# Digital-Defiance/node-fhe-accelerate

Hardware: AMD Instinct MI355X
Metric: NTTs/s at degree 16384 (batched, forward NTT + pointwise modmul) (higher is better)
Workload: dtype u64 (32-bit Shoup/Montgomery lanes for q<2^30); 1 GPU; C3: N=16384 forward NTT + modmul, batch 65536 per GPU, q=132120577; n=16384, batch_per_gpu=65536, global_batch=65536, q=132120577, parallelism=batch-sharded x1, no data-path collective

## Files before the change

node-fhe-accelerate_amd/csrc/fhe_arith.hpp:

```cpp
#pragma once
#ifndef FHE_NS
#define FHE_NS fhe
#endif
#include <hip/hip_runtime.h>
#include <stdint.h>

namespace FHE_NS {

__device__ __forceinline__ uint32_t mulhi(uint32_t a, uint32_t b) { return __umulhi(a, b); }
#ifndef FHE_MULHI64
#define FHE_MULHI64 3
#endif
__device__ __forceinline__ uint64_t mulhi(uint64_t a, uint64_t b) {
#if FHE_MULHI64 == 4
    const uint32_t a0 = (uint32_t)a, a1 = (uint32_t)(a >> 32), b0 = (uint32_t)b, b1 = (uint32_t)(b >> 32);
    const uint64_t m1 = (uint64_t)a1 * b0 + (uint64_t)__umulhi(a0, b0);
    const uint64_t m2 = (uint64_t)a0 * b1 + (uint64_t)(uint32_t)m1;
    const uint64_t h = (uint64_t)a1 * b1 + (m1 >> 32);
    return h + (m2 >> 32);
#elif FHE_MULHI64 == 3
    const uint32_t a0 = (uint32_t)a, a1 = (uint32_t)(a >> 32), b0 = (uint32_t)b, b1 = (uint32_t)(b >> 32);
    const uint64_t m1 = (uint64_t)a1 * b0 + __umulhi(a0, b0);
    uint64_t m2, cy;
    asm("v_mad_u64_u32 %0, %1, %2, %3, %4" : "=&v"(m2), "=&s"(cy) : "v"(a0), "v"(b1), "v"(m1));
// ... 158 lines not shown
        u32x2 cc;
        cc.x = c;
        uint64_t r, cy;
        asm("v_mad_u64_u32 %0, %1, %2, %3, %4" : "=&v"(r), "=&s"(cy) : "v"(a), "v"(b), "v"(cc));
        (void)cy;
        return (uint32_t)r;
    }
    static __device__ __forceinline__ uint32_t madlo_s(uint32_t a, uint32_t b, uint32_t c) {
        typedef uint32_t u32x2 __attribute__((ext_vector_type(2)));
        u32x2 cc;
        cc.x = c;
        uint64_t r, cy;
        asm("v_mad_u64_u32 %0, %1, %2, %3, %4" : "=&v"(r), "=&s"(cy) : "v"(a), "s"(b), "v"(cc));
        (void)cy;
        return (uint32_t)r;
    }
    template <int SP = 0>
    __device__ __forceinline__ W shoup(W x, Tw<W> t) const { return shoup<true, SP>(x, t.w, t.wp); }
    template <int SP = 0>
    __device__ __forceinline__ W shoup_inv(W x, Tw<W> t) const { return shoup<false, SP>(x, t.w, t.wp); }

    __device__ __forceinline__ W mont(W a, W b) const {
        W lo = a * b;
        W hi = mulhi(a, b);
        if constexpr (sizeof(W) == 8 && FHE_U64_NOVCC) {
            const W m = lo * (W(0) - qinv);
            return (W)sub_add64(hi, mulhi(m, q), (uint64_t)q + 1);
        } else {
            W m = lo * qinv;
            return hi + mulhi(m, q) + (lo != 0 ? W(1) : W(0));
        }
    }

    __device__ __forceinline__ W red2q(W x) const { return redk(x, q2); }
    __device__ __forceinline__ W red1q(W x) const { return redk(x, q); }
    static __device__ __forceinline__ W redk(W x, W k) {
        if constexpr (sizeof(W) == 8 && FHE_U64_NOVCC) {
            return (W)redk64(x, k);
        } else if constexpr (sizeof(W) == 8 && FHE_RED64_BORROW) {
            W d;
            return __builtin_sub_overflow(x, k, &d) ? x : d;
        } else {
            return umin(x, W(x - k));
        }
    }
    __device__ __forceinline__ W canon4(W x) const { return red1q(red2q(x)); }

    __device__ __forceinline__ W shoup_neg(W y, Tw<W> t) const {
        const W h = mulhi(y, t.wp);
        typedef uint32_t u32x2 __attribute__((ext_vector_type(2)));
        u32x2 c;
        c.x = y * t.w;
        uint64_t r, cy;
        asm("v_mad_u64_u32 %0, %1, %2, %3, %4" : "=&v"(r), "=&s"(cy) : "v"(h), "s"(q), "v"(c));
        (void)cy;
        return (W)r;
    }
    template <int SP = 0>
    __device__ __forceinline__ void ct(W &x, W &y, Tw<W> t) const {
        W a = red2q(x);
        if constexpr (sizeof(W) == 4 && FHE_NEG_FWD_TW) {
            const W nb = shoup_neg(y, t);
            x = a - nb;
            y = a + nb + q2;
        } else {
            W b = shoup<SP>(y, t);
// ... 19 lines not shown
        }
    }
    template <int SP = 0>
    __device__ __forceinline__ void ct_rscale(W &x, W &y, Scale<W> r) const {
        W a = shoup<SP>(x, r.a);
        W b = shoup<SP>(y, r.b);
        x = a + b;
        y = sub2q(a, b);
    }
    __device__ __forceinline__ void ct_unit(W &x, W &y) const {
        const W a = red2q(x), b = red2q(y);
        x = a + b;
        y = sub2q(a, b);
    }
    __device__ __forceinline__ void gs_unit(W &x, W &y) const {
        const W s = x + y, d = sub2q(x, y);
        x = red2q(s);
        y = red2q(d);
    }
    template <int SP = 0>
    __device__ __forceinline__ void gs(W &x, W &y, Tw<W> t) const {
        W s = x + y;
        W d = sub2q(x, y);
        x = red2q(s);
        y = shoup_inv<SP>(d, t);
    }
    template <int SP = 0>
    __device__ __forceinline__ void gs_scaled(W &x, W &y, Scale<W> ninv) const {
        W s = x + y;
        W d = sub2q(x, y);
        x = shoup_inv<SP>(s, ninv.a);
        y = shoup_inv<SP>(d, ninv.b);
    }
};

__device__ __forceinline__ uint64_t mod64_slow(uint64_t x, uint64_t q, uint64_t mu) {
    if (q >> 63) return x >= q ? x - q : x;
    uint64_t r = x - __umul64hi(x, mu) * q;
    return r >= q ? r - q : r;
}

__device__ __forceinline__ uint64_t wmont(uint64_t a, uint64_t b, uint64_t q, uint64_t qinv) {
    const uint64_t lo = a * b, hi = __umul64hi(a, b);
    const uint64_t mh = __umul64hi(lo * qinv, q);
    const uint64_t s = hi + mh;
    const bool c1 = s < hi;
    const uint64_t s2 = s + (lo != 0);
    const bool c2 = s2 < s;
    return (c1 || c2 || s2 >= q) ? s2 - q : s2;
}
__device__ __forceinline__ uint64_t wadd(uint64_t a, uint64_t b, uint64_t q) {
    const uint64_t s = a + b;
    return (s < a || s >= q) ? s - q : s;
}
__device__ __forceinline__ uint64_t wsub(uint64_t a, uint64_t b, uint64_t q) { return a >= b ? a - b : a - b + q; }
template <typename W>
__device__ __forceinline__ W load_lazy(uint64_t x, uint64_t lim, uint64_t q, uint64_t mu) {
    if (x >= lim) x = mod64_slow(x, q, mu);
    return W(x);
}

}
```

node-fhe-accelerate_amd/csrc/fhe_gpu.cpp:

```cpp
#include <hip/hip_runtime.h>

#include <algorithm>
#include <cstdlib>
#include <cstdio>
#include <cstring>
#include <mutex>
#include <thread>
#include <string>
#include <vector>

#include "../../include/fhe_gpu.h"
#include "fhe_internal.hpp"
#include "keygen.hpp"
#include "build_id.h"

using u64 = uint64_t;
using u32 = uint32_t;
using u128 = unsigned __int128;

namespace {

thread_local std::string g_err;

int fail(int code, const std::string &msg) {
// ... 772 lines not shown
            if (e != hipSuccess) { rc = hip_fail(e, "hipMalloc(big-N scratch)"); break; }
        }
    }
    if (rc == FHE_OK) {
        hipError_t e = hipStreamCreateWithFlags(&c->own_stream, hipStreamNonBlocking);
        if (e != hipSuccess) rc = hip_fail(e, "hipStreamCreate");
    }
    if (rc == FHE_OK) {
        const char *kv = std::getenv("FHE_POOL_KEEP_MB");
        const uint64_t keep_mb = kv ? std::strtoull(kv, nullptr, 10) : 8192;
        hipMemPool_t pool = nullptr;
        if (keep_mb && hipDeviceGetDefaultMemPool(&pool, device) == hipSuccess && pool) {
            uint64_t keep = keep_mb << 20;
            (void)hipMemPoolSetAttribute(pool, hipMemPoolAttrReleaseThreshold, &keep);
        }
        (void)hipGetLastError();
    }
    if (rc != FHE_OK) {
        free_tables(c);
        delete c;
        return rc;
    }
    c->stream = c->own_stream;
    c->plan.logn = logn;
    c->plan.word = c->word;
    {
        int cus = 0;
        if (hipDeviceGetAttribute(&cus, hipDeviceAttributeMultiprocessorCount, device) != hipSuccess || cus <= 0) cus = 256;
        (void)hipGetLastError();
        c->plan.cus = cus;
    }
    c->plan.wide = c->wide;
    c->plan.lazy = c->word == 32 && (u128)(4 + 2 * logn) * q <= ((u128)1 << 32);
    {
        const char *u = std::getenv("FHE_UNIT_TW");
        c->plan.compat = c->mode == FHE_MODE_COMPAT && !(u && u[0] == '0');
    }
    c->plan.stream = c->stream;
    c->plan.big_sync = &c->big_sync;
    *out = c;
    return FHE_OK;
}

int fhe_ctx_create_multi(uint32_t n, uint64_t q, int mode, const int *devices, int ndev, fhe_ctx **out) {
    if (!out) return fail(FHE_ERR_INVALID_ARG, "null out");
    *out = nullptr;
    if (!devices || ndev < 1) return fail(FHE_ERR_INVALID_ARG, "at least one device required");
    fhe_ctx *m = new fhe_ctx();
    for (int i = 0; i < ndev; ++i) {
        fhe_ctx *s = nullptr;
        const int rc = fhe_ctx_create(n, q, mode, devices[i], &s);
        if (rc != FHE_OK) {
            const std::string msg = g_err;
            fhe_ctx_destroy(m);
            return fail(rc, msg);
        }
        m->subs.push_back(s);
    }
    const fhe_ctx *s0 = m->subs[0];
    m->n = s0->n; m->logn = s0->logn; m->q = s0->q; m->psi = s0->psi; m->psi_inv = s0->psi_inv;
    m->inv_n = s0->inv_n; m->mode = s0->mode; m->device = s0->device; m->word = s0->word;
    m->fwd_tw = s0->fwd_tw; m->inv_tw = s0->inv_tw;
    m->stream = s0->stream;
    *out = m;
    return FHE_OK;
}
// ... 647 lines not shown
    FHE_TRY(hs.map(where, lwe_b, batch * 8, 1));
    FHE_TRY(hs.map(where, values, batch * 8, 2));
    FHE_TRY(hs.map(where, phase, batch * 8, 2));
    HIP_TRY(FHE_NS::launch_lwe_decrypt(q, t, sk, dim, lwe_a, lwe_b, values, phase, batch, s), "lwe decrypt kernel");
    return where == FHE_HOST ? hs.finish() : FHE_OK;
}

struct fhe_rns_ctx {
    std::vector<fhe_ctx *> limbs;
    void *tab = nullptr;
    FHE_NS::ModConsts *mtab = nullptr;
};

int fhe_rns_ctx_create(uint32_t n, const uint64_t *moduli, uint32_t count, int mode, int device, fhe_rns_ctx **out) {
    if (!out) return fail(FHE_ERR_INVALID_ARG, "null out");
    *out = nullptr;
    if (count == 0 || !moduli) return fail(FHE_ERR_INVALID_ARG, "At least one modulus required");
    fhe_rns_ctx *r = new fhe_rns_ctx();
    for (uint32_t i = 0; i < count; ++i) {
        fhe_ctx *c = nullptr;
        const int rc = fhe_ctx_create(n, moduli[i], mode, device, &c);
        if (rc != FHE_OK) {
            const std::string msg = g_err;
            fhe_rns_ctx_destroy(r);
            return fail(rc, msg);
        }
        if (!r->limbs.empty()) fhe_ctx_set_stream(c, r->limbs[0]->stream);
        r->limbs.push_back(c);
    }
    const fhe_ctx *c0 = r->limbs[0];
    bool one = !c0->plan.wide && (int)c0->logn <= FHE_NS::kMaxFusedLogN;
    for (const fhe_ctx *c : r->limbs)
        one = one && !c->plan.wide && c->plan.word == c0->plan.word && c->plan.lazy == c0->plan.lazy &&
              c->logn == c0->logn && c->device == c0->device;
    if (one) {
        DeviceGuard g(c0->device);
        const size_t L = r->limbs.size();
        std::vector<FHE_NS::ModConsts> mc(L);
        for (size_t i = 0; i < L; ++i) mc[i] = mod_consts(r->limbs[i]->q);
        std::vector<char> at;
        if (c0->plan.word == 32) {
            at.resize(L * sizeof(FHE_NS::NttArgs<uint32_t>));
            for (size_t i = 0; i < L; ++i)
                std::memcpy(at.data() + i * sizeof(FHE_NS::NttArgs<uint32_t>), &r->limbs[i]->plan.a32,
                            sizeof(FHE_NS::NttArgs<uint32_t>));
        } else {
            at.resize(L * sizeof(FHE_NS::NttArgs<uint64_t>));
            for (size_t i = 0; i < L; ++i)
                std::memcpy(at.data() + i * sizeof(FHE_NS::NttArgs<uint64_t>), &r->limbs[i]->plan.a64,
                            sizeof(FHE_NS::NttArgs<uint64_t>));
        }
        hipError_t e = hipMalloc(&r->tab, at.size());
        if (e == hipSuccess) e = hipMalloc((void **)&r->mtab, L * sizeof(FHE_NS::ModConsts));
        if (e == hipSuccess) e = hipMemcpy(r->tab, at.data(), at.size(), hipMemcpyHostToDevice);
        if (e == hipSuccess) e = hipMemcpy(r->mtab, mc.data(), L * sizeof(FHE_NS::ModConsts), hipMemcpyHostToDevice);
        if (e != hipSuccess) {
            fhe_rns_ctx_destroy(r);
            return hip_fail(e, "hipMalloc(RNS limb tables)");
        }
    }
    *out = r;
    return FHE_OK;
}

void fhe_rns_ctx_destroy(fhe_rns_ctx *r) {
    if (!r) return;
    if (r->tab || r->mtab) {
// ... 713 lines not shown
```

node-fhe-accelerate_amd/csrc/fhe_internal.hpp:

```cpp
#pragma once
#include <hip/hip_runtime.h>
#include <stddef.h>
#include <stdint.h>

#include <mutex>

#include "ntt_core.hpp"

namespace FHE_NS {

struct BigSync {
    std::mutex mu;
    hipEvent_t done = nullptr;
    hipStream_t last = nullptr;
};

struct WideArgs {
    const uint64_t *twf, *twi;
    uint64_t q, qinv, mu;
    uint64_t r2;
    uint64_t ninv_m;
    uint64_t ninv_r2;
};

struct Plan {
    uint32_t logn;
    int word;
    int wide;
    int lazy;
    int compat;
    int cus;
    hipStream_t stream;
    uint64_t *big_scratch[2];
    size_t big_chunk;
    BigSync *big_sync;
    NttArgs<uint32_t> a32;
    NttArgs<uint64_t> a64;
    WideArgs wa;
};

constexpr int kMinLogN = 2;
constexpr int kMaxFusedLogN = 14;
constexpr int kMaxLogN = 16;

hipError_t launch_fwd(const Plan &p, const uint64_t *in, uint64_t *out, size_t batch, int epi);
hipError_t launch_inv(const Plan &p, const uint64_t *in, uint64_t *out, size_t batch);
hipError_t launch_fwd_mul(const Plan &p, const uint64_t *a, const uint64_t *w, uint64_t *out, size_t batch);
hipError_t launch_polymul(const Plan &p, const uint64_t *a, const uint64_t *b, uint64_t *c, size_t batch);
hipError_t launch_fwd_limbs(const Plan &p, const void *tab, int limbs, const uint64_t *in, uint64_t *out,
                            size_t batch);
hipError_t launch_inv_limbs(const Plan &p, const void *tab, int limbs, const uint64_t *a, const uint64_t *b,
                            uint64_t *c, size_t batch);
hipError_t launch_wide(const Plan &p, int op, const uint64_t *a, const uint64_t *b, uint64_t *c, size_t batch);
hipError_t launch_big(const Plan &p, int op, const uint64_t *a, const uint64_t *b, uint64_t *c, size_t batch);
hipError_t launch_extprod(const Plan &p, int k1, int level, int base_log, const uint64_t *glwe,
                          const uint64_t *ggsw, uint64_t *out, size_t batch);
bool extprod_acc_supported(const Plan &p, int k1, int level, int base_log);
hipError_t launch_extprod_acc(const Plan &p, int level, int base_log, const uint64_t *glwe, const uint64_t *ggsw,
                              uint64_t *out, size_t batch);

hipError_t launch_relin(const Plan &p, int level, int base_log, const uint64_t *ct3, const uint64_t *rlk,
                        uint64_t *out, size_t batch);
// ... 85 lines not shown
```

node-fhe-accelerate_amd/csrc/ntt_core.hpp:

```cpp
#pragma once
#include "fhe_arith.hpp"

namespace FHE_NS {

constexpr int kPadA[17] = {0, 0, 0, 0, 0, 3, 3, 3, 4, 5, 5, 6, 7, 8, 5, 5, 0};
constexpr int kPadB[17] = {0, 0, 0, 0, 0, 0, 0, 0, 0, 0, 0, 0, 0, 0, 10, 10, 0};

constexpr int gk(int logn, int loge) { return logn | (loge << 8); }
constexpr int gk_logn(int k) { return k & 0xff; }
constexpr int gk_loge(int k) { return ((k >> 8) & 0xf) ? ((k >> 8) & 0xf) : ((k & 0xff) < 4 ? (k & 0xff) : 4); }
constexpr int gk_sparse(int k, int sel) { return k | (sel << 12); }
constexpr int gk_sp(int k) { return (k >> 12) & 3; }
constexpr int gk_compat(int k) { return k | (1 << 14); }
constexpr bool gk_cp(int k) { return (k >> 14) & 1; }

constexpr int pad_a(int L, int E) {
    return E == 5 ? 0 : (L == 10 && E == 3) ? 5 : (L == 10 && E == 2) ? 4 : kPadA[L];
}
constexpr int pad_b(int L, int E) {
    return E == 5 ? L - 5 : (L == 10 && E == 3) ? 6 : (L == 10 && E == 2) ? 5 : kPadB[L];
}
template <int K>
__host__ __device__ constexpr uint32_t pad_idx(uint32_t i) {
    constexpr int L = gk_logn(K);
    constexpr int A = pad_a(L, gk_loge(K));
    constexpr int B = pad_b(L, gk_loge(K));
    return i + (A ? (i >> A) : 0u) + (B ? (i >> B) : 0u);
}
template <int K>
constexpr int lds_words() { return (int)pad_idx<K>((1u << gk_logn(K)) - 1) + 1; }

#ifndef FHE_SPLIT_X64
#define FHE_SPLIT_X64 0
#endif
template <int K, typename W>
constexpr bool split_x() { return FHE_SPLIT_X64 && sizeof(W) == 8 && gk_logn(K) >= 14 && gk_loge(K) == 5; }
template <int K, typename W>
constexpr int lds_elems() { return split_x<K, W>() ? (lds_words<K>() + 1) / 2 : lds_words<K>(); }

template <int LOGN>
struct Geo {
    static constexpr int L = gk_logn(LOGN);
    static constexpr int N = 1 << L;
    static constexpr int LOGE = gk_loge(LOGN);
    static constexpr int E = 1 << LOGE;
    static constexpr int LOGT = L - LOGE;
    static constexpr int T = 1 << LOGT;
// ... 208 lines not shown
                    t[P::slot(k, u, tl)] = Tw<W>{cp[2 * idx], cp[2 * idx + 1]};
                } else if constexpr (G::P == 1) {
                    constexpr uint32_t m = (1u << S) - 1;
                    const uint32_t cst = (1u << (S + k)) + ((uint32_t(u) << G::LOGT) & m) + (uint32_t(tl) << S);
                    t[P::slot(k, u, tl)] = bload_tw<W>(brsrc(tw), (tau & m) * (uint32_t)sizeof(Tw<W>),
                                                       cst * (uint32_t)sizeof(Tw<W>));
                } else
                    t[P::slot(k, u, tl)] = tw[idx];
            }
    }
}

template <int LOGN, int PASS, int K, bool LAZY, typename W, bool RS = false>
__device__ __forceinline__ void fwd_stage(W (&v)[Geo<LOGN>::E], const Tw<W> (&t)[PassTw<LOGN, PASS>::COUNT],
                                          const Arith<W> &ar, Scale<W> rmod = Scale<W>{}) {
    using P = PassTw<LOGN, PASS>;
    constexpr int R = P::R, NU = P::NU;
#pragma unroll
    for (int u = 0; u < NU; ++u)
#pragma unroll
        for (int tt = 0; tt < (1 << R); ++tt) {
            if (tt & (1 << K)) continue;
            const int e = tt + (u << R), e2 = e + (1 << K);
            constexpr bool UNIT = gk_cp(LOGN) && PASS == 0 && (!LAZY || K == 0);
            if constexpr (RS && PASS == 0 && K == 0) ar.template ct_rscale<gk_sp(LOGN)>(v[e], v[e2], rmod);
            else if (UNIT && (tt & ((1 << K) - 1)) == 0) ar.ct_unit(v[e], v[e2]);
            else {
                const Tw<W> w = t[P::slot(K, u, tt & ((1 << K) - 1))];
                if constexpr (LAZY) ar.template ct_lazy<gk_sp(LOGN)>(v[e], v[e2], w);
                else ar.template ct<gk_sp(LOGN)>(v[e], v[e2], w);
            }
        }
}
template <int LOGN, int PASS, int K, bool FOLD, typename W>
__device__ __forceinline__ void inv_stage(W (&v)[Geo<LOGN>::E], const Tw<W> (&t)[PassTw<LOGN, PASS>::COUNT],
                                          const Arith<W> &ar, Scale<W> scale) {
    using P = PassTw<LOGN, PASS>;
    constexpr int S = P::S, R = P::R, NU = P::NU;
#pragma unroll
    for (int u = 0; u < NU; ++u)
#pragma unroll
        for (int tt = 0; tt < (1 << R); ++tt) {
            if (tt & (1 << K)) continue;
            const int e = tt + (u << R), e2 = e + (1 << K);
            if constexpr (FOLD && S + K == 0) ar.template gs_scaled<gk_sp(LOGN)>(v[e], v[e2], scale);
            else if (gk_cp(LOGN) && PASS == 0 && (tt & ((1 << K) - 1)) == 0) ar.gs_unit(v[e], v[e2]);
            else ar.template gs<gk_sp(LOGN)>(v[e], v[e2], t[P::slot(K, u, tt & ((1 << K) - 1))]);
        }
}
template <int LOGN, int PASS, int K, bool LAZY, bool RS, typename W>
__device__ __forceinline__ void fwd_stages_from(W (&v)[Geo<LOGN>::E], const Tw<W> (&t)[PassTw<LOGN, PASS>::COUNT],
                                                const Arith<W> &ar, Scale<W> rmod) {
    if constexpr (K < PassTw<LOGN, PASS>::R) {
        fwd_stage<LOGN, PASS, K, LAZY, W, RS>(v, t, ar, rmod);
        fwd_stages_from<LOGN, PASS, K + 1, LAZY, RS>(v, t, ar, rmod);
    }
}
template <int LOGN, int PASS, int K, bool FOLD, typename W>
__device__ __forceinline__ void inv_stages_from(W (&v)[Geo<LOGN>::E], const Tw<W> (&t)[PassTw<LOGN, PASS>::COUNT],
                                                const Arith<W> &ar, Scale<W> scale) {
    if constexpr (K >= 0) {
        inv_stage<LOGN, PASS, K, FOLD>(v, t, ar, scale);
        inv_stages_from<LOGN, PASS, K - 1, FOLD>(v, t, ar, scale);
    }
}
template <int LOGN, int PASS, bool LAZY, typename W, bool RS = false>
__device__ __forceinline__ void fwd_pass(W (&v)[Geo<LOGN>::E], const Tw<W> (&t)[PassTw<LOGN, PASS>::COUNT],
                                         const Arith<W> &ar, Scale<W> rmod = Scale<W>{}) {
    fwd_stages_from<LOGN, PASS, 0, LAZY, RS>(v, t, ar, rmod);
}
template <int LOGN, int PASS, bool FOLD, typename W>
__device__ __forceinline__ void inv_pass(W (&v)[Geo<LOGN>::E], const Tw<W> (&t)[PassTw<LOGN, PASS>::COUNT],
                                         const Arith<W> &ar, Scale<W> scale) {
    inv_stages_from<LOGN, PASS, PassTw<LOGN, PASS>::R - 1, FOLD>(v, t, ar, scale);
}

struct NoHook {
    __device__ void operator()() const {}
};

template <int LOGN, int PASS, int K, int LOOK, bool LAZY, typename W>
__device__ __forceinline__ void fwd_stages(uint32_t tau, W (&v)[Geo<LOGN>::E], Tw<W> (&t)[PassTw<LOGN, PASS>::COUNT],
                                           const Tw<W> *__restrict__ tw, const Arith<W> &ar) {
    constexpr int R = PassTw<LOGN, PASS>::R;
    if constexpr (K < R) {
        if constexpr (K + LOOK < R) load_tw<LOGN, PASS, W, K + LOOK, K + LOOK + 1>(tau, tw, t);
        fwd_stage<LOGN, PASS, K, LAZY>(v, t, ar);
        __builtin_amdgcn_sched_barrier(0);
        fwd_stages<LOGN, PASS, K + 1, LOOK, LAZY>(tau, v, t, tw, ar);
    }
}
template <int LOGN, int PASS, int K, int LOOK, bool FOLD, typename W>
__device__ __forceinline__ void inv_stages(uint32_t tau, W (&v)[Geo<LOGN>::E], Tw<W> (&t)[PassTw<LOGN, PASS>::COUNT],
                                           const Tw<W> *__restrict__ tw, const Arith<W> &ar, Scale<W> scale) {
    if constexpr (K >= 0) {
        if constexpr (K - LOOK >= 0) load_tw<LOGN, PASS, W, K - LOOK, K - LOOK + 1>(tau, tw, t);
        inv_stage<LOGN, PASS, K, FOLD>(v, t, ar, scale);
        __builtin_amdgcn_sched_barrier(0);
        inv_stages<LOGN, PASS, K - 1, LOOK, FOLD>(tau, v, t, tw, ar, scale);
    }
}
template <int LOGN>
constexpr bool staged_tw() { return Geo<LOGN>::LOGE >= 5; }

#ifndef FHE_STREAM_TW
#define FHE_STREAM_TW 1
#endif
#ifndef FHE_STREAM_DEPTH
#define FHE_STREAM_DEPTH 4
#endif
template <int LOGN, typename W>
constexpr bool stream_tw() { return FHE_STREAM_TW && sizeof(W) == 8 && Geo<LOGN>::LOGE == 5; }
#ifndef FHE_STREAM_TW2
#define FHE_STREAM_TW2 0
#endif
template <int LOGN, typename W>
constexpr bool stream_tw2() { return FHE_STREAM_TW2 && Geo<LOGN>::LOGE == 5; }
constexpr int kStreamDepth = FHE_STREAM_DEPTH;
#ifndef FHE_STREAM_PRE
#define FHE_STREAM_PRE 1
#endif

struct SItem { int k, u, tl; };
__host__ __device__ constexpr SItem stream_item(int R, int NU, bool inv, int i) {
    for (int s = 0; s < R; ++s) {
        const int k = inv ? R - 1 - s : s;
        if (i < NU << k) return SItem{k, i >> k, i & ((1 << k) - 1)};
        i -= NU << k;
    }
    return SItem{0, 0, 0};
}

// ... 122 lines not shown
    constexpr int R = PassTw<LOGN, PASS>::R;
    if constexpr (K < R) {
        if constexpr (K + LOOK < R) load_tw<LOGN, PASS, W, K + LOOK, K + LOOK + 1>(tau, tw, t);
        fwd_stage<LOGN, PASS, K, LAZY>(v, t, ar);
        fwd_stage<LOGN, PASS, K, LAZY>(v2, t, ar);
        __builtin_amdgcn_sched_barrier(0);
        fwd_stages2<LOGN, PASS, K + 1, LOOK, LAZY>(tau, v, v2, t, tw, ar);
    }
}
template <int LOGN, int PASS, bool LAZY, int PF, typename W>
__device__ __forceinline__ void fwd_rest2(W *lds, W (&v)[Geo<LOGN>::E], W (&v2)[Geo<LOGN>::E], uint32_t tau,
                                          const Tw<W> *__restrict__ tw, const Arith<W> &ar) {
    using G = Geo<LOGN>;
    if constexpr (PASS < G::NP) {
        Tw<W> t[PassTw<LOGN, PASS>::COUNT];
        if constexpr (stream_tw2<LOGN, W>()) {
            stream_begin<LOGN, PASS, false, false>(tau, tw, t);
            exchange<LOGN, PASS - 1, PASS>(lds, v, tau);
            xbar<lab_local<PASS - 1, PASS>()>();
            exchange<LOGN, PASS - 1, PASS>(lds, v2, tau);
            fwd_pass_stream<LOGN, PASS, LAZY, false, true>(tau, v, t, tw, ar, Scale<W>{}, &v2);
            fwd_rest2<LOGN, PASS + 1, LAZY, PF>(lds, v, v2, tau, tw, ar);
            return;
        }
        load_tw<LOGN, PASS, W, 0, PF>(tau, tw, t);
        exchange<LOGN, PASS - 1, PASS>(lds, v, tau);
        xbar<lab_local<PASS - 1, PASS>()>();
        exchange<LOGN, PASS - 1, PASS>(lds, v2, tau);
        fwd_stages2<LOGN, PASS, 0, PF, LAZY>(tau, v, v2, t, tw, ar);
        fwd_rest2<LOGN, PASS + 1, LAZY, PF>(lds, v, v2, tau, tw, ar);
    }
}

template <int LOGN, int PASS, bool FOLD, int PF, typename W>
__device__ __forceinline__ void inv_rest(W *lds, W (&v)[Geo<LOGN>::E], uint32_t tau, const Tw<W> *__restrict__ tw,
                                         const Arith<W> &ar, Scale<W> scale) {
    if constexpr (PASS >= 0) {
        Tw<W> t[PassTw<LOGN, PASS>::COUNT];
        if constexpr (stream_tw<LOGN, W>()) {
            if constexpr (FHE_STREAM_PRE) stream_begin<LOGN, PASS, true, FOLD && PASS == 0>(tau, tw, t);
            exchange<LOGN, PASS + 1, PASS>(lds, v, tau);
            if constexpr (!FHE_STREAM_PRE) stream_begin<LOGN, PASS, true, FOLD && PASS == 0>(tau, tw, t);
            inv_pass_stream<LOGN, PASS, FOLD>(tau, v, t, tw, ar, scale);
            inv_rest<LOGN, PASS - 1, FOLD, PF>(lds, v, tau, tw, ar, scale);
            return;
        }
        constexpr int R = PassTw<LOGN, PASS>::R;
        constexpr int KS = R - PF < 0 ? 0 : R - PF;
        load_tw<LOGN, PASS, W, KS, 8>(tau, tw, t);
        exchange<LOGN, PASS + 1, PASS>(lds, v, tau);
        if constexpr (staged_tw<LOGN>()) {
            inv_stages<LOGN, PASS, R - 1, R - KS, FOLD>(tau, v, t, tw, ar, scale);
        } else {
            load_tw<LOGN, PASS, W, 0, KS>(tau, tw, t);
            inv_pass<LOGN, PASS, FOLD>(v, t, ar, scale);
        }
        inv_rest<LOGN, PASS - 1, FOLD, PF>(lds, v, tau, tw, ar, scale);
    }
}

template <typename W>
struct NttArgs {
    const Tw<W> *twf;
    const Tw<W> *twi;
    Arith<W> ar;
    uint64_t q64, mu64;
    Scale<W> ninv;
    Scale<W> ninv_r;
    Scale<W> rs;
    Tw<W> rmod;
    Tw<W> one;
};

template <bool LAZY, typename W>
__device__ __forceinline__ W fwd_to_2q(W x, const NttArgs<W> &A) {
    if constexpr (LAZY) return A.ar.shoup(x, A.one);
    else return A.ar.red2q(x);
}
template <bool LAZY, typename W>
__device__ __forceinline__ W fwd_to_canon(W x, const NttArgs<W> &A) {
    return A.ar.red1q(fwd_to_2q<LAZY>(x, A));
}

template <typename W>
struct SlowRed {
    const NttArgs<W> &A;
    __device__ __forceinline__ uint64_t operator()(uint64_t x) const {
        if constexpr (sizeof(W) == 4) {
            const W r = A.ar.shoup((W)(x >> 32), A.rmod) + A.ar.shoup((W)x, A.one);
            return (uint64_t)A.ar.canon4(r);
// ... 132 lines not shown
    using G = Geo<LOGN>;
    static_assert(G::P == 1, "dual transform: one polynomial pair per workgroup");
    constexpr bool ST = stream_tw2<LOGN, W>();
    const Tw<W> *const twf = opaque_tw(A.twf);
    Tw<W> t0[PassTw<LOGN, 0>::COUNT];
    if constexpr (!ST) load_tw<LOGN, 0>(tau, twf, t0);
    const uint64_t lim = (uint64_t)(A.ar.q2 * 2);
    const uint32_t vo = tau * 8u;
    {
        const auto r = brsrc(src);
        load_coeffs_chunked<G::E, FHE_POLY2_CH, FHE_LOAD_INFLIGHT>(v, lim, SlowRed<W>{A}, [&](int t) -> uint64_t {
            return bload(r, vo, cbrv(t, G::LOGE) * G::T * 8u);
        });
    }
    {
        const auto r = brsrc(src2);
        load_coeffs_chunked<G::E, FHE_POLY2_CH, FHE_LOAD_INFLIGHT>(v2, lim, SlowRed<W>{A}, [&](int t) -> uint64_t {
            return bload(r, vo, cbrv(t, G::LOGE) * G::T * 8u);
        });
    }
    if constexpr (ST) {
        stream_begin<LOGN, 0, false, false>(tau, twf, t0);
        fwd_pass_stream<LOGN, 0, LAZY, false, true>(tau, v, t0, twf, A.ar, Scale<W>{}, &v2);
    } else {
        fwd_pass<LOGN, 0, LAZY, W>(v, t0, A.ar);
        fwd_pass<LOGN, 0, LAZY, W>(v2, t0, A.ar);
    }
    fwd_rest2<LOGN, 1, LAZY, PF>(lds, v, v2, tau, twf, A.ar);
}

struct NoFin {
    __device__ uint64_t operator()(uint32_t, uint64_t x) const { return x; }
};
template <int LOGN, int PF = kPfSingle, bool STORE = true, typename W, typename F = NoFin>
__device__ __forceinline__ void inv_poly_from_regs(W *lds, W (&v)[Geo<LOGN>::E], uint32_t tau, uint64_t *__restrict__ dst,
                                                   bool valid, const NttArgs<W> &A, Scale<W> scale, uint32_t sh = 0,
                                                   F &&fin = NoFin{}) {
    using G = Geo<LOGN>;
    constexpr int LAST = G::NP - 1;
    const Tw<W> *const twi = opaque_tw(A.twi);
    {
        Tw<W> t[PassTw<LOGN, LAST>::COUNT];
        if constexpr (stream_tw<LOGN, W>()) {
            stream_begin<LOGN, LAST, true, false>(tau, twi, t);
            inv_pass_stream<LOGN, LAST, true>(tau, v, t, twi, A.ar, scale);
        } else {
            load_tw<LOGN, LAST>(tau, twi, t);
            inv_pass<LOGN, LAST, true>(v, t, A.ar, scale);
        }
    }
    inv_rest<LOGN, LAST - 1, true, PF>(lds, v, tau, twi, A.ar, scale);
#pragma unroll
    for (int t = 0; t < G::E; ++t) {
        const uint32_t gi = (tau + cbrv(t, G::LOGE) * G::T) << sh;
        const uint64_t y = fin(gi, (uint64_t)A.ar.red1q(v[t]));
        if constexpr (!STORE) (void)y;
        else if constexpr (G::P == 1)
            bstore(brsrc(dst), (tau << sh) * 8u, ((cbrv(t, G::LOGE) * G::T) << sh) * 8u, y);
        else if (valid)
            __builtin_nontemporal_store(y, dst + gi);
    }
}

template <int LOGN, int PASS, int K, int LOOK, bool FOLD, typename W>
__device__ __forceinline__ void inv_stages2(uint32_t tau, W (&v)[Geo<LOGN>::E], W (&v2)[Geo<LOGN>::E],
                                            Tw<W> (&t)[PassTw<LOGN, PASS>::COUNT], const Tw<W> *__restrict__ tw,
                                            const Arith<W> &ar, Scale<W> scale) {
    if constexpr (K >= 0) {
        if constexpr (K - LOOK >= 0) load_tw<LOGN, PASS, W, K - LOOK, K - LOOK + 1>(tau, tw, t);
        inv_stage<LOGN, PASS, K, FOLD>(v, t, ar, scale);
        inv_stage<LOGN, PASS, K, FOLD>(v2, t, ar, scale);
        __builtin_amdgcn_sched_barrier(0);
        inv_stages2<LOGN, PASS, K - 1, LOOK, FOLD>(tau, v, v2, t, tw, ar, scale);
    }
}
template <int LOGN, int PASS, bool FOLD, int PF, typename W>
__device__ __forceinline__ void inv_rest2(W *lds, W (&v)[Geo<LOGN>::E], W (&v2)[Geo<LOGN>::E], uint32_t tau,
                                          const Tw<W> *__restrict__ tw, const Arith<W> &ar, Scale<W> scale) {
    if constexpr (PASS >= 0) {
        Tw<W> t[PassTw<LOGN, PASS>::COUNT];
        if constexpr (stream_tw2<LOGN, W>()) {
            stream_begin<LOGN, PASS, true, FOLD && PASS == 0>(tau, tw, t);
            exchange<LOGN, PASS + 1, PASS>(lds, v, tau);
            xbar<lab_local<PASS + 1, PASS>()>();
            exchange<LOGN, PASS + 1, PASS>(lds, v2, tau);
            inv_pass_stream<LOGN, PASS, FOLD, true>(tau, v, t, tw, ar, scale, &v2);
            inv_rest2<LOGN, PASS - 1, FOLD, PF>(lds, v, v2, tau, tw, ar, scale);
            return;
        }
        constexpr int R = PassTw<LOGN, PASS>::R;
        constexpr int KS = R - PF < 0 ? 0 : R - PF;
        load_tw<LOGN, PASS, W, KS, 8>(tau, tw, t);
        exchange<LOGN, PASS + 1, PASS>(lds, v, tau);
        xbar<lab_local<PASS + 1, PASS>()>();
// ... 37 lines not shown
```

node-fhe-accelerate_amd/csrc/ntt_inv.hip:

```cpp
#ifndef FHE_SPLIT_X64
#define FHE_SPLIT_X64 1
#endif
#ifndef FHE_U64_NOVCC
#define FHE_U64_NOVCC 1
#endif
#ifndef FHE_MULHI64
#define FHE_MULHI64 4
#endif
#include "fhe_internal.hpp"

namespace FHE_NS {

template <int LOGN, typename W>
__device__ __forceinline__ void ntt_inv_body(const uint64_t *__restrict__ in, uint64_t *__restrict__ out, size_t batch,
                                             const NttArgs<W> &A) {
    using G = Geo<LOGN>;
    __shared__ W lds_all[G::P * lds_elems<LOGN, W>()];
    const uint32_t tau = threadIdx.x & (G::T - 1), pl = wg_poly<G>();
    const size_t poly = (size_t)blockIdx.x * G::P + pl;
    const bool valid = poly < batch;
    W *lds = lds_all + pl * lds_elems<LOGN, W>();
    if (G::P == 1 && !valid) return;
    W v[G::E];
    const uint64_t *src = in + poly * G::N;
// ... 137 lines not shown
#pragma unroll
    for (int e = 0; e < G::E; ++e) {
        const uint32_t gi = gidx<LOGN, G::NP - 1>(tb, e);
        W x;
        if constexpr (STASH == 0) x = va[e];
        else if constexpr (STASH == 1) x = st[gi];
        else x = valid ? reinterpret_cast<const W *>(crow)[gi] : W(0);
        v[e] = A.ar.mont(x, v[e]);
    }
    if constexpr (G::NP > 1) __syncthreads();
    uint32_t ti = tau;
    if constexpr (sizeof(W) == 8 || STASH == 2) asm volatile("" : "+v"(ti));
    inv_poly_from_regs<LOGN, polymul_pf<LOGN>()>(lds, v, ti, crow, valid, A, A.ninv_r);
}
template <int LOGN, typename W, bool LAZY>
__global__ void __launch_bounds__(Geo<LOGN>::THREADS, (polymul_occ<LOGN, W>()))
k_polymul(const uint64_t *__restrict__ a, const uint64_t *__restrict__ b, uint64_t *c, size_t batch,
          NttArgs<W> A) {
    polymul_body<LOGN, W, LAZY>(a, b, c, batch, A);
}
template <int LOGN, typename W, bool LAZY>
__global__ void __launch_bounds__(Geo<LOGN>::THREADS)
k_polymul_limbs(const uint64_t *__restrict__ a, const uint64_t *__restrict__ b, uint64_t *c, size_t batch,
                const NttArgs<W> *__restrict__ tab) {
    const size_t o = (size_t)blockIdx.y * batch * Geo<LOGN>::N;
    const NttArgs<W> A = tab[blockIdx.y];
    polymul_body<LOGN, W, LAZY>(a + o, b + o, c + o, batch, A);
}

#ifndef FHE_POLY_LAB
#define FHE_POLY_LAB 0
#endif
template <int LOGN, typename W, bool LAZY>
__device__ __forceinline__ void polymul2_one(W *lds, uint32_t tau, const uint64_t *__restrict__ a,
                                             const uint64_t *__restrict__ b, uint64_t *c, size_t poly,
                                             const NttArgs<W> &A) {
    using G = Geo<LOGN>;
    W v[G::E], vb[G::E];
    fwd_poly2<LOGN, LAZY, polymul2_pf<LOGN, W>()>(lds, v, vb, tau, a + poly * G::N, b + poly * G::N, A);
#pragma unroll
    for (int e = 0; e < G::E; ++e) v[e] = A.ar.mont(fwd_to_canon<LAZY>(v[e], A), vb[e]);
    __syncthreads();
    inv_poly_from_regs<LOGN, polymul2_pf<LOGN, W>()>(lds, v, tau, c + poly * G::N, true, A, A.ninv_r);
}

template <int LOGN, typename W>
constexpr int polymul2_occ() {
    constexpr int o = Geo<LOGN>::template occ_waves<W>();
    return (FHE_POLY_DUAL_E16 && Geo<LOGN>::LOGE == 4 && (sizeof(W) == 4 || gk_logn(LOGN) < 14) && o > 4) ? 4 : o;
}
template <int LOGN, typename W, bool LAZY>
__global__ void __launch_bounds__(Geo<LOGN>::THREADS, (polymul2_occ<LOGN, W>()))
k_polymul2(const uint64_t *__restrict__ a, const uint64_t *__restrict__ b, uint64_t *c, size_t batch,
           NttArgs<W> A) {
    using G = Geo<LOGN>;
    static_assert(G::P == 1, "one polynomial pair per workgroup");
    __shared__ W lds[lds_elems<LOGN, W>()];
    const uint32_t tau = threadIdx.x;
    const size_t poly = blockIdx.x;
    if (poly >= batch) return;
#if FHE_POLY_LAB == 1
    {
        const auto ra = brsrc(a + poly * G::N), rb = brsrc(b + poly * G::N), rc = brsrc(c + poly * G::N);
#pragma unroll
        for (int ch = 0; ch < G::E; ch += 8) {
            uint64_t x[8];
#pragma unroll
            for (int e = 0; e < 8; ++e) x[e] = bload(ra, tau * 8u, (ch + e) * G::T * 8u) ^ bload(rb, tau * 8u, (ch + e) * G::T * 8u);
#pragma unroll
            for (int e = 0; e < 8; ++e) bstore(rc, tau * 8u, (ch + e) * G::T * 8u, x[e]);
        }
        return;
// ... 23 lines not shown
#endif
    polymul2_one<LOGN, W, LAZY>(lds, tau, a, b, c, poly, A);
}
template <int LOGN, typename W, bool LAZY>
__global__ void __launch_bounds__(Geo<LOGN>::THREADS)
k_polymul2_limbs(const uint64_t *__restrict__ a, const uint64_t *__restrict__ b, uint64_t *c, size_t batch,
                 const NttArgs<W> *__restrict__ tab) {
    __shared__ W lds[lds_elems<LOGN, W>()];
    const size_t poly = blockIdx.x;
    if (poly >= batch) return;
    const size_t o = (size_t)blockIdx.y * batch * Geo<LOGN>::N;
    const NttArgs<W> A = tab[blockIdx.y];
    polymul2_one<LOGN, W, LAZY>(lds, threadIdx.x, a + o, b + o, c + o, poly, A);
}

template <int LOGN, typename W>
static hipError_t inv_one(const Plan &p, const NttArgs<W> &A, hipStream_t s, const uint64_t *a, const uint64_t *b,
                          uint64_t *c, size_t batch, const NttArgs<W> *tab = nullptr, int limbs = 1) {
    auto go = [&](auto K, auto KL, size_t blocks, int threads, auto... args) -> hipError_t {
        if (tab)
            hipLaunchKernelGGL(KL, dim3((unsigned)blocks, (unsigned)limbs), dim3(threads), 0, s, args..., tab);
        else
            hipLaunchKernelGGL(K, dim3((unsigned)blocks), dim3(threads), 0, s, args..., A);
        return hipGetLastError();
    };
    bool lazy = false;
    if constexpr (sizeof(W) == 4) lazy = p.lazy;
    constexpr int PK = polymul_key<LOGN, W>();
    using GP = Geo<PK>;
    size_t pblocks = (batch + GP::P - 1) / GP::P;
    if constexpr (polymul_dual<PK, W>()) {
        if (b) {
            if constexpr (sizeof(W) == 4) {
                if (lazy)
                    return go(k_polymul2<PK, W, true>, k_polymul2_limbs<PK, W, true>, pblocks, GP::THREADS, a, b, c,
                              batch);
            }
            if constexpr (sizeof(W) == 8) {
                if (!tab && A.ar.sp == 1 && p.compat)
                    return go(k_polymul2<gk_compat(gk_sparse(PK, 1)), W, false>, k_polymul2_limbs<PK, W, false>,
                              pblocks, GP::THREADS, a, b, c, batch);
                if (!tab && A.ar.sp == 1)
                    return go(k_polymul2<gk_sparse(PK, 1), W, false>, k_polymul2_limbs<PK, W, false>, pblocks,
                              GP::THREADS, a, b, c, batch);
                if (!tab && A.ar.sp == 2)
                    return go(k_polymul2<gk_sparse(PK, 2), W, false>, k_polymul2_limbs<PK, W, false>, pblocks,
                              GP::THREADS, a, b, c, batch);
                if (!tab && p.compat)
                    return go(k_polymul2<gk_compat(PK), W, false>, k_polymul2_limbs<PK, W, false>, pblocks,
                              GP::THREADS, a, b, c, batch);
            }
            return go(k_polymul2<PK, W, false>, k_polymul2_limbs<PK, W, false>, pblocks, GP::THREADS, a, b, c, batch);
        }
    } else {
        if (b && lazy) {
            if constexpr (sizeof(W) == 4)
                return go(k_polymul<PK, W, true>, k_polymul_limbs<PK, W, true>, pblocks, GP::THREADS, a, b, c, batch);
            return hipErrorInvalidValue;
        } else if (b) {
            return go(k_polymul<PK, W, false>, k_polymul_limbs<PK, W, false>, pblocks, GP::THREADS, a, b, c, batch);
        }
    }
    constexpr int IK = inv_key<LOGN, W>();
    using GI = Geo<IK>;
    const size_t iblocks = (batch + GI::P - 1) / GI::P;
    return go(k_ntt_inv<IK, W>, k_ntt_inv_limbs<IK, W>, iblocks, GI::THREADS, a, c, batch);
}

template <typename W>
// ... 58 lines not shown
```

Before: 14.92 million NTTs/s.

## Add compile-time lazy-reduction schedule for inverse NTT in fused polymul

```diff
diff --git a/node-fhe-accelerate_amd/csrc/fhe_arith.hpp b/node-fhe-accelerate_amd/csrc/fhe_arith.hpp
--- a/node-fhe-accelerate_amd/csrc/fhe_arith.hpp
+++ b/node-fhe-accelerate_amd/csrc/fhe_arith.hpp
@@ -214,6 +214,13 @@
         }
     }
 
+    __device__ __forceinline__ W mont_signed(W a, W b) const {
+        static_assert(sizeof(W) == 4, "32-bit words");
+        const W lo = a * b, hi = mulhi(a, b);
+        const W m = lo * (W(0) - qinv);
+        return hi - mulhi(m, q) + q;
+    }
+
     __device__ __forceinline__ W red2q(W x) const { return redk(x, q2); }
     __device__ __forceinline__ W red1q(W x) const { return redk(x, q); }
     static __device__ __forceinline__ W redk(W x, W k) {
@@ -299,6 +306,18 @@
         x = shoup_inv<SP>(s, ninv.a);
         y = shoup_inv<SP>(d, ninv.b);
     }
+    __device__ __forceinline__ void gs_lazy(W &x, W &y, W kq, Tw<W> t) const {
+        const W s = x + y;
+        const W d = x - y + kq;
+        x = s;
+        y = shoup_inv(d, t);
+    }
+    __device__ __forceinline__ void gs_scaled_lazy(W &x, W &y, W kq, Scale<W> ninv) const {
+        const W s = x + y;
+        const W d = x - y + kq;
+        x = shoup_inv(s, ninv.a);
+        y = shoup_inv(d, ninv.b);
+    }
 };
 
 __device__ __forceinline__ uint64_t mod64_slow(uint64_t x, uint64_t q, uint64_t mu) {
diff --git a/node-fhe-accelerate_amd/csrc/fhe_gpu.cpp b/node-fhe-accelerate_amd/csrc/fhe_gpu.cpp
--- a/node-fhe-accelerate_amd/csrc/fhe_gpu.cpp
+++ b/node-fhe-accelerate_amd/csrc/fhe_gpu.cpp
@@ -828,6 +828,10 @@
     }
     c->plan.wide = c->wide;
     c->plan.lazy = c->word == 32 && (u128)(4 + 2 * logn) * q <= ((u128)1 << 32);
+    {
+        const char *li = std::getenv("FHE_LAZY_INV");
+        c->plan.lazy_inv = c->word == 32 && (u128)32 * q <= ((u128)1 << 32) && !(li && li[0] == '0');
+    }
     {
         const char *u = std::getenv("FHE_UNIT_TW");
         c->plan.compat = c->mode == FHE_MODE_COMPAT && !(u && u[0] == '0');
@@ -1541,7 +1545,7 @@
     bool one = !c0->plan.wide && (int)c0->logn <= FHE_NS::kMaxFusedLogN;
     for (const fhe_ctx *c : r->limbs)
         one = one && !c->plan.wide && c->plan.word == c0->plan.word && c->plan.lazy == c0->plan.lazy &&
-              c->logn == c0->logn && c->device == c0->device;
+              c->plan.lazy_inv == c0->plan.lazy_inv && c->logn == c0->logn && c->device == c0->device;
     if (one) {
         DeviceGuard g(c0->device);
         const size_t L = r->limbs.size();
diff --git a/node-fhe-accelerate_amd/csrc/fhe_internal.hpp b/node-fhe-accelerate_amd/csrc/fhe_internal.hpp
--- a/node-fhe-accelerate_amd/csrc/fhe_internal.hpp
+++ b/node-fhe-accelerate_amd/csrc/fhe_internal.hpp
@@ -28,6 +28,7 @@
     int word;
     int wide;
     int lazy;
+    int lazy_inv;
     int compat;
     int cus;
     hipStream_t stream;
diff --git a/node-fhe-accelerate_amd/csrc/lazy_inv_sched.hpp b/node-fhe-accelerate_amd/csrc/lazy_inv_sched.hpp
--- /dev/null
+++ b/node-fhe-accelerate_amd/csrc/lazy_inv_sched.hpp
@@ -0,0 +1,93 @@
+#pragma once
+#include <stdint.h>
+
+namespace linv {
+
+constexpr int kMaxPass = 4;
+constexpr int kMaxStage = 5;
+constexpr int kQBits = 27;
+constexpr int kLimit = 32;
+constexpr int kSlotsUmin = 3;
+constexpr int kSlotsShoup = 4;
+
+struct Sched {
+    int logn, loge, np, entry, b;
+    int r[kMaxPass];
+    uint32_t umin[kMaxPass][kMaxStage], shp[kMaxPass][kMaxStage];
+    uint32_t kq[kMaxPass][kMaxStage][4];
+    uint32_t xumin[kMaxPass], xshp[kMaxPass];
+    int n_umin[kMaxPass], n_shp[kMaxPass];
+    int max_bound;
+    int slots;
+    bool ok;
+};
+
+constexpr int pow2_ge(int x) {
+    int k = 2;
+    while (k < x) k *= 2;
+    return k;
+}
+constexpr bool fits(int bx, int by) { return bx + by <= kLimit && bx + pow2_ge(by) <= kLimit && pow2_ge(by) <= 16; }
+constexpr int red_slots(int b) { return b <= 2 ? 0 : (b <= 4 ? kSlotsUmin : kSlotsShoup); }
+
+constexpr Sched make(int logn, int loge, int entry, int B) {
+    Sched s{};
+    s.logn = logn; s.loge = loge; s.entry = entry; s.b = B;
+    s.np = (logn + loge - 1) / loge;
+    s.ok = s.np <= kMaxPass && loge <= kMaxStage && entry >= 1 && entry <= kLimit;
+    if (!s.ok) return s;
+    const int E = 1 << loge;
+    int bd[32] = {};
+    for (int e = 0; e < E; ++e) bd[e] = entry;
+    s.max_bound = entry;
+    auto reduce = [&](int p, int e, uint32_t &mu, uint32_t &ms) {
+        if (bd[e] <= 2) return;
+        if (bd[e] <= 4) { mu |= 1u << e; ++s.n_umin[p]; }
+        else { ms |= 1u << e; ++s.n_shp[p]; }
+        s.slots += red_slots(bd[e]);
+        bd[e] = 2;
+    };
+    for (int p = s.np - 1; p >= 0; --p) {
+        const int R = (logn - p * loge) < loge ? (logn - p * loge) : loge;
+        s.r[p] = R;
+        for (int k = R - 1; k >= 0; --k) {
+            for (int e = 0; e < E; ++e) {
+                if (e & (1 << k)) continue;
+                const int e2 = e | (1 << k);
+                if (!fits(bd[e], bd[e2])) {
+                    const int cx = red_slots(bd[e]), cy = red_slots(bd[e2]);
+                    const bool fx = fits(2, bd[e2]) && bd[e] > 2, fy = fits(bd[e], 2) && bd[e2] > 2;
+                    if (fx && (!fy || cx <= cy)) reduce(p, e, s.umin[p][k], s.shp[p][k]);
+                    else if (fy) reduce(p, e2, s.umin[p][k], s.shp[p][k]);
+                    else { reduce(p, e, s.umin[p][k], s.shp[p][k]); reduce(p, e2, s.umin[p][k], s.shp[p][k]); }
+                }
+                const int K = pow2_ge(bd[e2]);
+                int j = 0;
+                while ((2 << j) < K) ++j;
+                s.kq[p][k][j] |= 1u << e;
+                const int sum = bd[e] + bd[e2], d = bd[e] + K;
+                if (sum > s.max_bound) s.max_bound = sum;
+                if (d > s.max_bound) s.max_bound = d;
+                if (p == 0 && k == 0) { bd[e] = 2; bd[e2] = 2; }
+                else { bd[e] = sum; bd[e2] = 2; }
+            }
+        }
+        if (p > 0) {
+            for (int e = 0; e < E; ++e) {
+                if (bd[e] > B) reduce(p, e, s.xumin[p], s.xshp[p]);
+                bd[e] = B;
+            }
+        }
+    }
+    s.ok = s.max_bound <= kLimit;
+    return s;
+}
+
+constexpr Sched best(int logn, int loge, int entry) {
+    const Sched a = make(logn, loge, entry, 2), b = make(logn, loge, entry, 4);
+    if (!b.ok) return a;
+    if (!a.ok) return b;
+    return b.slots < a.slots ? b : a;
+}
+
+}
diff --git a/node-fhe-accelerate_amd/csrc/ntt_core.hpp b/node-fhe-accelerate_amd/csrc/ntt_core.hpp
--- a/node-fhe-accelerate_amd/csrc/ntt_core.hpp
+++ b/node-fhe-accelerate_amd/csrc/ntt_core.hpp
@@ -1,5 +1,6 @@
 #pragma once
 #include "fhe_arith.hpp"
+#include "lazy_inv_sched.hpp"
 
 namespace FHE_NS {
 
@@ -13,6 +14,10 @@
 constexpr int gk_sp(int k) { return (k >> 12) & 3; }
 constexpr int gk_compat(int k) { return k | (1 << 14); }
 constexpr bool gk_cp(int k) { return (k >> 14) & 1; }
+constexpr int gk_geninv(int k) { return k | (1 << 15); }
+constexpr bool gk_gi(int k) { return (k >> 15) & 1; }
+template <int LOGN, int ENTRY>
+inline constexpr linv::Sched kLinv = linv::best(gk_logn(LOGN), gk_loge(LOGN), ENTRY);
 
 constexpr int pad_a(int L, int E) {
     return E == 5 ? 0 : (L == 10 && E == 3) ? 5 : (L == 10 && E == 2) ? 4 : kPadA[L];
@@ -287,11 +292,40 @@
             }
         }
 }
-template <int LOGN, int PASS, int K, bool FOLD, typename W>
+template <int E, typename W>
+__device__ __forceinline__ void linv_reduce(W (&v)[E], uint32_t mu, uint32_t ms, const Arith<W> &ar, Tw<W> one) {
+#pragma unroll
+    for (int e = 0; e < E; ++e) {
+        if ((mu >> e) & 1) v[e] = ar.red2q(v[e]);
+        else if ((ms >> e) & 1) v[e] = ar.shoup(v[e], one);
+    }
+}
+template <int LOGN, int PASS, int K, bool FOLD, typename W, int LZ = 0>
 __device__ __forceinline__ void inv_stage(W (&v)[Geo<LOGN>::E], const Tw<W> (&t)[PassTw<LOGN, PASS>::COUNT],
-                                          const Arith<W> &ar, Scale<W> scale) {
+                                          const Arith<W> &ar, Scale<W> scale, Tw<W> one = Tw<W>{}) {
     using P = PassTw<LOGN, PASS>;
     constexpr int S = P::S, R = P::R, NU = P::NU;
+    if constexpr (LZ != 0) {
+        static_assert(sizeof(W) == 4 && !gk_cp(LOGN) && FOLD, "lazy inverse: 32-bit words, no unit-twiddle keys");
+        static_assert(kLinv<LOGN, LZ>.ok && kLinv<LOGN, LZ>.max_bound <= linv::kLimit &&
+                          ((uint64_t)linv::kLimit << linv::kQBits) <= (1ull << 32),
+                      "a scheduled sum, d or exchange value could pass 2^32 at q < 2^27");
+        static_assert(kLinv<LOGN, LZ>.r[PASS] == R && kLinv<LOGN, LZ>.np == Geo<LOGN>::NP, "schedule / geometry mismatch");
+        constexpr uint32_t MU = kLinv<LOGN, LZ>.umin[PASS][K], MS = kLinv<LOGN, LZ>.shp[PASS][K];
+        constexpr uint32_t K0 = kLinv<LOGN, LZ>.kq[PASS][K][0], K1 = kLinv<LOGN, LZ>.kq[PASS][K][1],
+                           K2 = kLinv<LOGN, LZ>.kq[PASS][K][2];
+        linv_reduce(v, MU, MS, ar, one);
+#pragma unroll
+        for (int e = 0; e < Geo<LOGN>::E; ++e) {
+            if (e & (1 << K)) continue;
+            const int e2 = e + (1 << K);
+            const W kq = ((K0 >> e) & 1) ? ar.q2 : ((K1 >> e) & 1) ? W(ar.q2 * 2) : ((K2 >> e) & 1) ? W(ar.q2 * 4) : W(ar.q2 * 8);
+            if constexpr (S + K == 0) ar.gs_scaled_lazy(v[e], v[e2], kq, scale);
+            else ar.gs_lazy(v[e], v[e2], kq, t[P::slot(K, e >> R, e & ((1 << K) - 1))]);
+        }
+        if constexpr (K == 0 && PASS > 0) linv_reduce(v, kLinv<LOGN, LZ>.xumin[PASS], kLinv<LOGN, LZ>.xshp[PASS], ar, one);
+        return;
+    }
 #pragma unroll
     for (int u = 0; u < NU; ++u)
 #pragma unroll
@@ -311,12 +345,12 @@
         fwd_stages_from<LOGN, PASS, K + 1, LAZY, RS>(v, t, ar, rmod);
     }
 }
-template <int LOGN, int PASS, int K, bool FOLD, typename W>
+template <int LOGN, int PASS, int K, bool FOLD, typename W, int LZ = 0>
 __device__ __forceinline__ void inv_stages_from(W (&v)[Geo<LOGN>::E], const Tw<W> (&t)[PassTw<LOGN, PASS>::COUNT],
-                                                const Arith<W> &ar, Scale<W> scale) {
+                                                const Arith<W> &ar, Scale<W> scale, Tw<W> one = Tw<W>{}) {
     if constexpr (K >= 0) {
-        inv_stage<LOGN, PASS, K, FOLD>(v, t, ar, scale);
-        inv_stages_from<LOGN, PASS, K - 1, FOLD>(v, t, ar, scale);
+        inv_stage<LOGN, PASS, K, FOLD, W, LZ>(v, t, ar, scale, one);
+        inv_stages_from<LOGN, PASS, K - 1, FOLD, W, LZ>(v, t, ar, scale, one);
     }
 }
 template <int LOGN, int PASS, bool LAZY, typename W, bool RS = false>
@@ -324,10 +358,10 @@
                                          const Arith<W> &ar, Scale<W> rmod = Scale<W>{}) {
     fwd_stages_from<LOGN, PASS, 0, LAZY, RS>(v, t, ar, rmod);
 }
-template <int LOGN, int PASS, bool FOLD, typename W>
+template <int LOGN, int PASS, bool FOLD, typename W, int LZ = 0>
 __device__ __forceinline__ void inv_pass(W (&v)[Geo<LOGN>::E], const Tw<W> (&t)[PassTw<LOGN, PASS>::COUNT],
-                                         const Arith<W> &ar, Scale<W> scale) {
-    inv_stages_from<LOGN, PASS, PassTw<LOGN, PASS>::R - 1, FOLD>(v, t, ar, scale);
+                                         const Arith<W> &ar, Scale<W> scale, Tw<W> one = Tw<W>{}) {
+    inv_stages_from<LOGN, PASS, PassTw<LOGN, PASS>::R - 1, FOLD, W, LZ>(v, t, ar, scale, one);
 }
 
 struct NoHook {
@@ -345,14 +379,15 @@
         fwd_stages<LOGN, PASS, K + 1, LOOK, LAZY>(tau, v, t, tw, ar);
     }
 }
-template <int LOGN, int PASS, int K, int LOOK, bool FOLD, typename W>
+template <int LOGN, int PASS, int K, int LOOK, bool FOLD, typename W, int LZ = 0>
 __device__ __forceinline__ void inv_stages(uint32_t tau, W (&v)[Geo<LOGN>::E], Tw<W> (&t)[PassTw<LOGN, PASS>::COUNT],
-                                           const Tw<W> *__restrict__ tw, const Arith<W> &ar, Scale<W> scale) {
+                                           const Tw<W> *__restrict__ tw, const Arith<W> &ar, Scale<W> scale,
+                                           Tw<W> one = Tw<W>{}) {
     if constexpr (K >= 0) {
         if constexpr (K - LOOK >= 0) load_tw<LOGN, PASS, W, K - LOOK, K - LOOK + 1>(tau, tw, t);
-        inv_stage<LOGN, PASS, K, FOLD>(v, t, ar, scale);
+        inv_stage<LOGN, PASS, K, FOLD, W, LZ>(v, t, ar, scale, one);
         __builtin_amdgcn_sched_barrier(0);
-        inv_stages<LOGN, PASS, K - 1, LOOK, FOLD>(tau, v, t, tw, ar, scale);
+        inv_stages<LOGN, PASS, K - 1, LOOK, FOLD, W, LZ>(tau, v, t, tw, ar, scale, one);
     }
 }
 template <int LOGN>
@@ -541,9 +576,9 @@
     }
 }
 
-template <int LOGN, int PASS, bool FOLD, int PF, typename W>
+template <int LOGN, int PASS, bool FOLD, int PF, typename W, int LZ = 0>
 __device__ __forceinline__ void inv_rest(W *lds, W (&v)[Geo<LOGN>::E], uint32_t tau, const Tw<W> *__restrict__ tw,
-                                         const Arith<W> &ar, Scale<W> scale) {
+                                         const Arith<W> &ar, Scale<W> scale, Tw<W> one = Tw<W>{}) {
     if constexpr (PASS >= 0) {
         Tw<W> t[PassTw<LOGN, PASS>::COUNT];
         if constexpr (stream_tw<LOGN, W>()) {
@@ -559,12 +594,12 @@
         load_tw<LOGN, PASS, W, KS, 8>(tau, tw, t);
         exchange<LOGN, PASS + 1, PASS>(lds, v, tau);
         if constexpr (staged_tw<LOGN>()) {
-            inv_stages<LOGN, PASS, R - 1, R - KS, FOLD>(tau, v, t, tw, ar, scale);
+            inv_stages<LOGN, PASS, R - 1, R - KS, FOLD, W, LZ>(tau, v, t, tw, ar, scale, one);
         } else {
             load_tw<LOGN, PASS, W, 0, KS>(tau, tw, t);
-            inv_pass<LOGN, PASS, FOLD>(v, t, ar, scale);
-        }
-        inv_rest<LOGN, PASS - 1, FOLD, PF>(lds, v, tau, tw, ar, scale);
+            inv_pass<LOGN, PASS, FOLD, W, LZ>(v, t, ar, scale, one);
+        }
+        inv_rest<LOGN, PASS - 1, FOLD, PF, W, LZ>(lds, v, tau, tw, ar, scale, one);
     }
 }
 
@@ -763,10 +798,10 @@
 struct NoFin {
     __device__ uint64_t operator()(uint32_t, uint64_t x) const { return x; }
 };
-template <int LOGN, int PF = kPfSingle, bool STORE = true, typename W, typename F = NoFin>
-__device__ __forceinline__ void inv_poly_from_regs(W *lds, W (&v)[Geo<LOGN>::E], uint32_t tau, uint64_t *__restrict__ dst,
-                                                   bool valid, const NttArgs<W> &A, Scale<W> scale, uint32_t sh = 0,
-                                                   F &&fin = NoFin{}) {
+template <int LZ, int LOGN, int PF = kPfSingle, bool STORE = true, typename W, typename F = NoFin>
+__device__ __forceinline__ void inv_poly_from_regs_lz(W *lds, W (&v)[Geo<LOGN>::E], uint32_t tau, uint64_t *__restrict__ dst,
+                                                      bool valid, const NttArgs<W> &A, Scale<W> scale, uint32_t sh = 0,
+                                                      F &&fin = NoFin{}) {
     using G = Geo<LOGN>;
     constexpr int LAST = G::NP - 1;
     const Tw<W> *const twi = opaque_tw(A.twi);
@@ -777,10 +812,10 @@
             inv_pass_stream<LOGN, LAST, true>(tau, v, t, twi, A.ar, scale);
         } else {
             load_tw<LOGN, LAST>(tau, twi, t);
-            inv_pass<LOGN, LAST, true>(v, t, A.ar, scale);
-        }
-    }
-    inv_rest<LOGN, LAST - 1, true, PF>(lds, v, tau, twi, A.ar, scale);
+            inv_pass<LOGN, LAST, true, W, LZ>(v, t, A.ar, scale, A.one);
+        }
+    }
+    inv_rest<LOGN, LAST - 1, true, PF, W, LZ>(lds, v, tau, twi, A.ar, scale, A.one);
 #pragma unroll
     for (int t = 0; t < G::E; ++t) {
         const uint32_t gi = (tau + cbrv(t, G::LOGE) * G::T) << sh;
@@ -791,6 +826,13 @@
         else if (valid)
             __builtin_nontemporal_store(y, dst + gi);
     }
+}
+
+template <int LOGN, int PF = kPfSingle, bool STORE = true, typename W, typename F = NoFin>
+__device__ __forceinline__ void inv_poly_from_regs(W *lds, W (&v)[Geo<LOGN>::E], uint32_t tau, uint64_t *__restrict__ dst,
+                                                   bool valid, const NttArgs<W> &A, Scale<W> scale, uint32_t sh = 0,
+                                                   F &&fin = NoFin{}) {
+    inv_poly_from_regs_lz<0, LOGN, PF, STORE>(lds, v, tau, dst, valid, A, scale, sh, fin);
 }
 
 template <int LOGN, int PASS, int K, int LOOK, bool FOLD, typename W>
diff --git a/node-fhe-accelerate_amd/csrc/ntt_inv.hip b/node-fhe-accelerate_amd/csrc/ntt_inv.hip
--- a/node-fhe-accelerate_amd/csrc/ntt_inv.hip
+++ b/node-fhe-accelerate_amd/csrc/ntt_inv.hip
@@ -193,12 +193,21 @@
 #define FHE_POLY_LAB 0
 #endif
 template <int LOGN, typename W, bool LAZY>
+constexpr bool lazy_inv_key() { return LAZY && sizeof(W) == 4 && !gk_gi(LOGN); }
+template <int LOGN, typename W, bool LAZY>
 __device__ __forceinline__ void polymul2_one(W *lds, uint32_t tau, const uint64_t *__restrict__ a,
                                              const uint64_t *__restrict__ b, uint64_t *c, size_t poly,
                                              const NttArgs<W> &A) {
     using G = Geo<LOGN>;
     W v[G::E], vb[G::E];
     fwd_poly2<LOGN, LAZY, polymul2_pf<LOGN, W>()>(lds, v, vb, tau, a + poly * G::N, b + poly * G::N, A);
+    if constexpr (lazy_inv_key<LOGN, W, LAZY>()) {
+#pragma unroll
+        for (int e = 0; e < G::E; ++e) v[e] = A.ar.mont_signed(fwd_to_2q<LAZY>(v[e], A), vb[e]);
+        __syncthreads();
+        inv_poly_from_regs_lz<3, LOGN, polymul2_pf<LOGN, W>()>(lds, v, tau, c + poly * G::N, true, A, A.ninv_r);
+        return;
+    }
 #pragma unroll
     for (int e = 0; e < G::E; ++e) v[e] = A.ar.mont(fwd_to_canon<LAZY>(v[e], A), vb[e]);
     __syncthreads();
@@ -288,9 +297,12 @@
     if constexpr (polymul_dual<PK, W>()) {
         if (b) {
             if constexpr (sizeof(W) == 4) {
-                if (lazy)
+                if (lazy && p.lazy_inv)
                     return go(k_polymul2<PK, W, true>, k_polymul2_limbs<PK, W, true>, pblocks, GP::THREADS, a, b, c,
                               batch);
+                if (lazy)
+                    return go(k_polymul2<gk_geninv(PK), W, true>, k_polymul2_limbs<gk_geninv(PK), W, true>, pblocks,
+                              GP::THREADS, a, b, c, batch);
             }
             if constexpr (sizeof(W) == 8) {
                 if (!tab && A.ar.sp == 1 && p.compat)
```

Measured after the change: 14.90 million NTTs/s. Within noise of the previous version (-0.2%).
